# KhaoulaAguech/pl-fem-vectoriel

Measured on AMD Instinct MI355X. Metric: eigenmodes/sec (assembly+solve), 7-core P2 mesh, 10 modes; |Δn_eff| vs ref, higher is better.
Workload: dtype f64

## Files before the change

### pl_fem_vectoriel_amd/csrc/kernels_lanczos.hip

```cpp
#include <algorithm>
#include <cmath>
#include <functional>

#include "device.h"
#include "p2_element.h"

namespace plfem {
namespace {

typedef double v4d __attribute__((ext_vector_type(4)));
constexpr int CHUNK = PANEL_CHUNK;

__global__ __launch_bounds__(256) void k_scale_store(int64_t n, const double* __restrict__ w,
                                                     const double* __restrict__ bw, const double* __restrict__ beta2,
                                                     double* __restrict__ v, double* __restrict__ bv,
                                                     double* __restrict__ beta_out) {
  const double b2 = *beta2;
  const double beta = sqrt(fmax(b2, 0.0));
  const double inv = beta > 0.0 ? 1.0 / beta : 0.0;
  const int64_t i = (int64_t)blockIdx.x * 256 + threadIdx.x;
  if (i == 0 && beta_out) *beta_out = beta;
  if (i >= n) return;
  v[i] = w[i] * inv;
  bv[i] = bw[i] * inv;
}

__global__ __launch_bounds__(256) void k_axpby(int64_t n, double a, const double* __restrict__ x, double b,
                                               const double* __restrict__ y, double* __restrict__ z) {
  const int64_t i = (int64_t)blockIdx.x * 256 + threadIdx.x;
  if (i < n) z[i] = a * x[i] + b * y[i];
}

template <int P, int CW>
__global__ __launch_bounds__(256) void k_panel_dot_p(int64_t n, int ncols, int nchunks, const double* __restrict__ Pm,
                                                     const double* __restrict__ W, int64_t ldw,
                                                     double* __restrict__ partial) {
  const int c0 = (blockIdx.y * 4 + (threadIdx.x >> 6)) * CW;
  if (c0 >= ncols) return;
  const int lane = threadIdx.x & 63;
  const int64_t i0 = (int64_t)blockIdx.x * CHUNK;
  const int64_t i1 = min(n, i0 + CHUNK);
  const double* col[CW];
#pragma unroll
  for (int t = 0; t < CW; ++t) col[t] = Pm + (int64_t)min(c0 + t, ncols - 1) * n;
  double acc[CW][P];
#pragma unroll
  for (int t = 0; t < CW; ++t)
#pragma unroll
    for (int q = 0; q < P; ++q) acc[t][q] = 0.0;
  int64_t i = i0 + lane;
  for (; i + 64 < i1; i += 128) {
    double a[2][CW], w[2][P];
#pragma unroll
    for (int h = 0; h < 2; ++h) {
#pragma unroll
      for (int t = 0; t < CW; ++t) a[h][t] = col[t][i + 64 * h];
#pragma unroll
      for (int q = 0; q < P; ++q) w[h][q] = W[(int64_t)q * ldw + i + 64 * h];
    }
#pragma unroll
    for (int h = 0; h < 2; ++h)
#pragma unroll
      for (int t = 0; t < CW; ++t)
#pragma unroll
        for (int q = 0; q < P; ++q) acc[t][q] += a[h][t] * w[h][q];
  }
  for (; i < i1; i += 64) {
    double w[P];
#pragma unroll
    for (int q = 0; q < P; ++q) w[q] = W[(int64_t)q * ldw + i];
#pragma unroll
    for (int t = 0; t < CW; ++t) {
      const double a = col[t][i];
#pragma unroll
      for (int q = 0; q < P; ++q) acc[t][q] += a * w[q];
    }
  }
#pragma unroll
  for (int t = 0; t < CW; ++t) {
#pragma unroll
    for (int q = 0; q < P; ++q) {
      double v = acc[t][q];
      for (int off = 32; off >= 1; off >>= 1) v += __shfl_xor(v, off);
      if (lane == 0 && c0 + t < ncols) partial[((int64_t)(c0 + t) * P + q) * nchunks + blockIdx.x] = v;
    }
  }
}

__global__ __launch_bounds__(64) void k_panel_dot_finish_p(int P, int nchunks, const double* __restrict__ partial,
                                                           double* __restrict__ h, int ldh, double* __restrict__ hacc,
                                                           int ldacc) {
  const int cq = blockIdx.x;
  const int c = cq / P, q = cq % P;
  double acc = 0.0;
  for (int t = threadIdx.x; t < nchunks; t += 64) acc += partial[(int64_t)cq * nchunks + t];
  for (int off = 32; off >= 1; off >>= 1) acc += __shfl_xor(acc, off);
  if (threadIdx.x == 0) {
    h[c + (int64_t)q * ldh] = acc;
    if (hacc) hacc[c + (int64_t)q * ldacc] += acc;
  }
}

template <int P>
__global__ __launch_bounds__(256) void k_panel_axpy_p(int64_t n, int ncols, const double* __restrict__ Pm,
                                                      const double* __restrict__ H, int ldh, double* __restrict__ W,
                                                      int64_t ldw, double* __restrict__ wil, int N, int dpn) {
  extern __shared__ double sh[];
  for (int k = threadIdx.x; k < ncols * P; k += 256) sh[k] = H[(k / P) + (int64_t)(k % P) * ldh];
  __syncthreads();
  const int64_t i = (int64_t)blockIdx.x * 256 + threadIdx.x;
  if (i >= n) return;
  double acc[P];
#pragma unroll
  for (int q = 0; q < P; ++q) acc[q] = 0.0;
  for (int c = 0; c < ncols; ++c) {
    const double a = Pm[(int64_t)c * n + i];
#pragma unroll
    for (int q = 0; q < P; ++q) acc[q] += a * sh[c * P + q];
  }
  double w[P];
#pragma unroll
  for (int q = 0; q < P; ++q) {
    w[q] = W[(int64_t)q * ldw + i] - acc[q];
    W[(int64_t)q * ldw + i] = w[q];
  }
  if (wil) {
    const int comp = (int)(i / N), node = (int)(i - (int64_t)comp * N);
    double* d = wil + ((int64_t)node * dpn + comp) * P;
#pragma unroll
    for (int q = 0; q < P; ++q) d[q] = w[q];
  }
}


template <int P>
__global__ __launch_bounds__(FIRST_THREADS) void k_permute_dot_first(int64_t n2, int N, int nseg, int ncols, const int32_t* __restrict__ npos,
                                                          const double* __restrict__ xl, double* __restrict__ W, int64_t ldw,
                                                          const double* __restrict__ Pm, double* __restrict__ partial) {
  constexpr int CW = FIRST_COLS, V = CW * P, NT = FIRST_THREADS, NW = NT / 64;
  static_assert(V <= 64 && (V & (V - 1)) == 0 && FIRST_ROWS % NT == 0 && NW == 4, "multi_reduce<V>; whole rows per thread; four waves meet");
  __shared__ double red[NW][V];
  const int seg = blockIdx.x, wave = threadIdx.x >> 6, lane = threadIdx.x & 63;
  double acc[V];
#pragma unroll
  for (int v = 0; v < V; ++v) acc[v] = 0.0;
  const double* col[CW];
#pragma unroll
  for (int t = 0; t < CW; ++t) col[t] = Pm + (int64_t)min(t, ncols - 1) * n2;
  constexpr int RPT = FIRST_ROWS / NT;
  int64_t g[RPT];
  int pos[RPT];
  double a[RPT][CW], w[RPT][P];
#pragma unroll
  for (int j = 0; j < RPT; ++j) {
    g[j] = (int64_t)seg * FIRST_ROWS + j * NT + threadIdx.x;
    const bool on = g[j] < n2;
    const int c = on && g[j] >= N;
    pos[j] = on ? npos[(int)(g[j] - (int64_t)c * N)] : -1;
#pragma unroll
    for (int t = 0; t < CW; ++t) a[j][t] = on ? col[t][g[j]] : 0.0;
  }
#pragma unroll
  for (int j = 0; j < RPT; ++j) {
    const int c = g[j] >= N;
#pragma unroll
    for (int q = 0; q < P; ++q) w[j][q] = pos[j] >= 0 ? xl[((int64_t)pos[j] + c) * P + q] : 0.0;
  }
#pragma unroll
  for (int j = 0; j < RPT; ++j) {
    if (g[j] < n2) {
#pragma unroll
      for (int q = 0; q < P; ++q) W[(int64_t)q * ldw + g[j]] = w[j][q];
    }
#pragma unroll
    for (int t = 0; t < CW; ++t)
#pragma unroll
      for (int q = 0; q < P; ++q) acc[t * P + q] = fma(a[j][t], w[j][q], acc[t * P + q]);
  }
  multi_reduce<V, true>(acc, lane);
  if ((lane & (64 / V - 1)) == 0) red[wave][multi_reduce_index<V, true>(lane)] = acc[0];
  __syncthreads();
  if ((int)threadIdx.x < V) {
    const int v = threadIdx.x, t = v / P;
    if (t < ncols) partial[(int64_t)v * nseg + seg] = (red[0][v] + red[1][v]) + (red[2][v] + red[3][v]);
  }
}

template <int P>
__global__ __launch_bounds__(256) void k_axpy_first(int64_t n, int ncols, int nseg, const double* __restrict__ Pm,
                                                    const double* __restrict__ partial, double* __restrict__ Hout, int ldh,
                                                    double* __restrict__ W, int64_t ldw) {
  constexpr int CW = 8;
  __shared__ double sh[CW * P];
  {
    const int v = threadIdx.x >> 3, part = threadIdx.x & 7;
    double x = 0.0;
    if (v / P < ncols) {
      const double* pp = partial + (int64_t)v * nseg;
      int k = part;
      for (; k + 7 * 8 < nseg; k += 8 * 8) {
        double t[8];
#pragma unroll
        for (int u = 0; u < 8; ++u) t[u] = pp[k + 8 * u];
#pragma unroll
        for (int u = 0; u < 8; ++u) x += t[u];
      }
      for (; k < nseg; k += 8) x += pp[k];
    }
    x += __shfl_xor(x, 1, 8);
    x += __shfl_xor(x, 2, 8);
    x += __shfl_xor(x, 4, 8);
    if (part == 0) {
      sh[v] = x;
      if (blockIdx.x == 0 && v / P < ncols) Hout[(v / P) + (int64_t)(v % P) * ldh] = x;
    }
  }
  __syncthreads();
  const int64_t i = (int64_t)blockIdx.x * 256 + threadIdx.x;
  if (i >= n) return;
  double a[CW];
#pragma unroll
  for (int t = 0; t < CW; ++t) a[t] = Pm[(int64_t)min(t, ncols - 1) * n + i];
  double acc[P];
#pragma unroll
  for (int q = 0; q < P; ++q) acc[q] = 0.0;
#pragma unroll
  for (int t = 0; t < CW; ++t)
    if (t < ncols) {
#pragma unroll
      for (int q = 0; q < P; ++q) acc[q] = fma(a[t], sh[t * P + q], acc[q]);
    }
#pragma unroll
  for (int q = 0; q < P; ++q) W[(int64_t)q * ldw + i] -= acc[q];
}

template <int P>
__global__ __launch_bounds__(64 * P * P > 1024 ? 1024 : 64 * P * P) void k_chol_small(const double* __restrict__ G, int ldg, const double* __restrict__ partial,
                                                           int nchunks, double* __restrict__ Tblk, int ldT,
                                                           double* __restrict__ Rinv, int32_t* __restrict__ counters) {
  __shared__ double sG[P * P];
  if (G) {
    if (threadIdx.x < P * P) sG[threadIdx.x] = G[(threadIdx.x % P) + (int64_t)(threadIdx.x / P) * ldg];
  } else {
    const int lane = threadIdx.x & 63;
    for (int cq = threadIdx.x >> 6; cq < P * P; cq += blockDim.x >> 6) {
      const double* pp = partial + (int64_t)cq * nchunks;
      double acc = 0.0;
      int t = lane;
      for (; t + 7 * 64 < nchunks; t += 8 * 64) {
        double v[8];
#pragma unroll
        for (int u = 0; u < 8; ++u) v[u] = pp[t + 64 * u];
#pragma unroll
        for (int u = 0; u < 8; ++u) acc += v[u];
      }
      for (; t < nchunks; t += 64) acc += pp[t];
      for (int off = 32; off >= 1; off >>= 1) acc += __shfl_xor(acc, off);
      if (lane == 0) sG[(cq / P) + (cq % P) * P] = acc;
    }
  }
  __syncthreads();
  if (threadIdx.x != 0) return;
  ldg = P;
  G = sG;
  double R[P][P], X[P][P];
  for (int i = 0; i < P; ++i)
    for (int j = 0; j < P; ++j) { R[i][j] = 0.0; X[i][j] = 0.0; }
  for (int j = 0; j < P; ++j) {
    for (int i = 0; i <= j; ++i) {
      double v = 0.5 * (G[i + (int64_t)j * ldg] + G[j + (int64_t)i * ldg]);
      for (int k = 0; k < i; ++k) v -= R[k][i] * R[k][j];
      if (i == j) {
        if (!(v > 0.0)) { atomicAdd(&counters[2], 1); v = 1.0; }
        R[j][j] = sqrt(v);
      } else {
        R[i][j] = v / R[i][i];
      }
    }
  }
  for (int j = 0; j < P; ++j) {
    X[j][j] = 1.0 / R[j][j];
    for (int i = j - 1; i >= 0; --i) {
      double v = 0.0;
      for (int k = i + 1; k <= j; ++k) v -= R[i][k] * X[k][j];
      X[i][j] = v / R[i][i];
    }
  }
  for (int i = 0; i < P; ++i)
    for (int j = 0; j < P; ++j) {
      Tblk[i + (int64_t)j * ldT] = R[i][j];
      Rinv[i + j * P] = X[i][j];
    }
}

template <int P>
__global__ __launch_bounds__(256) void k_block_scale(int64_t n, const double* __restrict__ W, const double* __restrict__ BW,
                                                     int64_t ldw, const double* __restrict__ Rinv,
                                                     double* __restrict__ Vn, double* __restrict__ BVn, int64_t ldv,
                                                     const double* __restrict__ exp_src, int exp_n, double* __restrict__ exp_dst,
                                                     const int32_t* __restrict__ cnt_src, int32_t* __restrict__ cnt_dst,
                                                     double* __restrict__ bv_front, const int32_t* __restrict__ npos, int N) {
  __shared__ double X[P * P];
  if (threadIdx.x < P * P) X[threadIdx.x] = Rinv[threadIdx.x];
  if (blockIdx.x == 0 && exp_dst) {
    for (int t = threadIdx.x; t < exp_n; t += 256) exp_dst[t] = exp_src[t];
    if (threadIdx.x < 4) cnt_dst[threadIdx.x] = cnt_src[threadIdx.x];
  }
  __syncthreads();
  const int64_t i = (int64_t)blockIdx.x * 256 + threadIdx.x;
  if (i >= n) return;
  double w[P], bw[P];
#pragma unroll
  for (int q = 0; q < P; ++q) { w[q] = W[(int64_t)q * ldw + i]; bw[q] = BW[(int64_t)q * ldw + i]; }
  int64_t fo = -1;
  if (bv_front) {
    const int c = i >= N;
    const int pos = npos[(int)(i - (int64_t)c * N)];
    if (pos >= 0) fo = ((int64_t)pos + c) * P;
  }
#pragma unroll
  for (int q = 0; q < P; ++q) {
    double a = 0.0, b = 0.0;
#pragma unroll
    for (int k = 0; k <= q; ++k) { a += w[k] * X[k + q * P]; b += bw[k] * X[k + q * P]; }
    Vn[(int64_t)q * ldv + i] = a;
    BVn[(int64_t)q * ldv + i] = b;
    if (fo >= 0) bv_front[fo + q] = b;
  }
}

__global__ __launch_bounds__(256) void k_rotate(int64_t n, int m, int p, const double* __restrict__ V,
                                                const double* __restrict__ Smat, int ldS, double* __restrict__ out) {
  extern __shared__ double sS[];
  const int mpad = (m + 3) & ~3, ppad = (p + 15) & ~15;
  for (int k = threadIdx.x; k < mpad * ppad; k += 256) {
    int r = k / ppad, c = k % ppad;
    sS[k] = (r < m && c < p) ? Smat[(int64_t)c * ldS + r] : 0.0;
  }
  __syncthreads();
  const int wave = threadIdx.x >> 6, lane = threadIdx.x & 63;
  const int64_t i0 = ((int64_t)blockIdx.x * 4 + wave) * 16;
  if (i0 >= n) return;
  const int lr = lane & 15, lk = lane >> 4;
  const int64_t row = i0 + lr;
  const bool rv = row < n;
  for (int c0 = 0; c0 < ppad; c0 += 16) {
    v4d acc = (v4d){0.0, 0.0, 0.0, 0.0};
    for (int kk = 0; kk < mpad; kk += 4) {
      int k = kk + lk;
      double a = sS[k * ppad + c0 + lr];
      double b = (rv && k < m) ? V[(int64_t)k * n + row] : 0.0;
      acc = __builtin_amdgcn_mfma_f64_16x16x4f64(a, b, acc, 0, 0, 0);
    }
#pragma unroll
    for (int r = 0; r < 4; ++r) {
      int oc = c0 + lk + 4 * r;
      if (rv && oc < p) out[(int64_t)oc * n + row] = acc[r];
    }
  }
}

__global__ __launch_bounds__(256) void k_core_mask(int N, const double* __restrict__ doflocs,
                                                   const double* __restrict__ cores, int ncore,
                                                   const uint8_t* __restrict__ bmask, uint8_t* __restrict__ mask,
                                                   int32_t* __restrict__ counters) {
  const int i = blockIdx.x * 256 + threadIdx.x;
  bool counted = false;
  if (i < N) {
    const bool in = in_any_core(doflocs[i], doflocs[N + i], cores, ncore);
    mask[i] = in ? 1 : 0;
    counted = in && !bmask[i];
  }
  unsigned long long b = __ballot(counted);
  if ((threadIdx.x & 63) == 0 && b) atomicAdd(&counters[1], (int)__popcll(b));
}

constexpr int POST_MB = 4;
template <int DPN>
__global__ __launch_bounds__(256) void k_post_sums(int N, int k, int nblocks, const int32_t* __restrict__ rowptr,
                                                   const int32_t* __restrict__ colind, const double* __restrict__ dxx,
                                                   const double* __restrict__ dxy, const double* __restrict__ dyy,
                                                   const uint8_t* __restrict__ mask, const double* __restrict__ evecs,
                                                   double* __restrict__ partial) {
  constexpr int MB = POST_MB;
  const int mode0 = blockIdx.y * MB;
  const int nm = min(MB, k - mode0);
  const double* vx[MB];
#pragma unroll
  for (int j = 0; j < MB; ++j) vx[j] = evecs + (int64_t)min(mode0 + j, k - 1) * DPN * N;
// ... 367 lines not shown
```

### pl_fem_vectoriel_amd/csrc/kernels_sweep.hip

```cpp
#include <algorithm>

#include "device.h"

namespace plfem {
namespace {

struct SweepArgs {
  int leaf_level;
  int ldv;
  int sh;
  const int32_t *cinv0, *cinv1, *prow;
  const double* front;
  const double2* dinv2;
  double *fr, *u0, *u1, *ys, *xl;
};

template <int P, bool SOA>
__device__ __forceinline__ int sidx(int i, int u, int ldv) { return SOA ? u * ldv + i : i * P + u; }

template <int P>
struct FwdStage {
  double a[P], b0[P], b1[P];
  int c0, c1;
  __device__ __forceinline__ void request(const SweepArgs& A, int64_t np, int i, bool on) {
    c0 = c1 = -1;
#pragma unroll
    for (int u = 0; u < P; ++u) { a[u] = 0.0; b0[u] = 0.0; b1[u] = 0.0; }
    if (!on) return;
    const int64_t e = (2 * np + i) * P;
#pragma unroll
    for (int u = 0; u < P; ++u) a[u] = A.fr[e + u];
    if (!A.leaf_level) {
      c0 = A.cinv0[np + (i >> A.sh)];
      c1 = A.cinv1[np + (i >> A.sh)];
#pragma unroll
      for (int u = 0; u < P; ++u) { b0[u] = A.u0[e + u]; b1[u] = A.u1[e + u]; }
    }
  }
  __device__ __forceinline__ double value(int u) const {
    return a[u] + (c0 >= 0 ? b0[u] : 0.0) + (c1 >= 0 ? b1[u] : 0.0);
  }
};

template <int P, bool SOA>
__device__ __forceinline__ void stage_fwd(const SweepArgs& A, double* sv, int64_t np, int need, int T, int tid,
                                          FwdStage<P>& first) {
  for (int i = tid + T; i < need; i += T) {
    FwdStage<P> s;
    s.request(A, np, i, true);
#pragma unroll
    for (int u = 0; u < P; ++u) sv[sidx<P, SOA>(i, u, A.ldv)] = s.value(u);
  }
  first.request(A, np, tid, tid < need);
}

template <int P>
struct FwdOut {
  double w0[P], w1[P];
  int c0, c1;
  int64_t dst;
  __device__ __forceinline__ void request(const SweepArgs& A, int64_t npp, int64_t np, int s2, int m, int r) {
    c0 = c1 = -1;
    dst = -1;
#pragma unroll
    for (int u = 0; u < P; ++u) { w0[u] = 0.0; w1[u] = 0.0; }
    if (r >= m || r < s2) return;
    const int pr = A.prow[np + (r >> A.sh)];
    if (!A.leaf_level) {
      c0 = A.cinv0[np + (r >> A.sh)];
      c1 = A.cinv1[np + (r >> A.sh)];
      const int64_t e = (2 * np + r) * P;
#pragma unroll
      for (int u = 0; u < P; ++u) { w0[u] = A.u0[e + u]; w1[u] = A.u1[e + u]; }
    }
    if (pr >= 0) dst = (2 * npp + (pr << A.sh) + (r & A.sh)) * P;
  }
  __device__ __forceinline__ double w(int u) const { return (c0 >= 0 ? w0[u] : 0.0) + (c1 >= 0 ? w1[u] : 0.0); }
};

template <int P, int NW, int TBF>
__device__ __forceinline__ void fwd_tile_body(const SweepArgs& A, const SweepJob& J, double* __restrict__ sv, double* __restrict__ red) {
  const int f = J.f, m = J.m, s2 = J.s2;
  const int r0 = (J.rb & ~SWEEP_ROW_JOB_FLAG) * 64;
  const int64_t np = J.np;
  const int tid = threadIdx.x, wave = tid >> 6, lane = tid & 63;
  const int need = (r0 + 64 <= s2) ? r0 + 64 : s2;
  const int r = r0 + lane;
  const bool valid = r < m;
  const int h = lane >> 5, ra = r0 + 2 * (lane & 31), rb = ra + 1;
  const bool pvalid = ra < m;
  const int cea = pvalid ? ((ra < s2) ? ra + 1 : s2) : 0;
  const int ceb = pvalid ? ((rb < s2) ? rb + 1 : s2) : 0;
  const double* p = A.front + J.foff + ra;
  FwdOut<P> out;
  if (wave == 0) out.request(A, J.npp, np, s2, m, r);
  FwdStage<P> st;
  stage_fwd<P, false>(A, sv, np, need, NW * 64, tid, st);
  double2 a0[TBF];
#pragma unroll
  for (int t = 0; t < TBF; ++t) {
    const int c = 2 * (wave + NW * t) + h;
    a0[t] = (c < ceb) ? *reinterpret_cast<const double2*>(p + (int64_t)c * m) : make_double2(0.0, 0.0);
  }
  if (tid < need) {
#pragma unroll
    for (int u = 0; u < P; ++u) sv[tid * P + u] = st.value(u);
  }
  __syncthreads();
  double acc[2][P];
#pragma unroll
  for (int u = 0; u < P; ++u) { acc[0][u] = 0.0; acc[1][u] = 0.0; }
#pragma unroll
  for (int t = 0; t < TBF; ++t) {
    const int c = 2 * (wave + NW * t) + h;
    if (c < ceb) {
      const double ax = (c < cea) ? a0[t].x : 0.0;
#pragma unroll
      for (int u = 0; u < P; ++u) {
        const double v = sv[c * P + u];
        acc[0][u] += ax * v;
        acc[1][u] += a0[t].y * v;
      }
    }
  }
  for (int c0 = 2 * NW * TBF; c0 < ceb; c0 += 2 * NW * TBF) {
    double2 a[TBF];
#pragma unroll
    for (int t = 0; t < TBF; ++t) {
      const int c = c0 + 2 * (wave + NW * t) + h;
      a[t] = (c < ceb) ? *reinterpret_cast<const double2*>(p + (int64_t)c * m) : make_double2(0.0, 0.0);
    }
#pragma unroll
    for (int t = 0; t < TBF; ++t) {
      const int c = c0 + 2 * (wave + NW * t) + h;
      if (c < ceb) {
        const double ax = (c < cea) ? a[t].x : 0.0;
#pragma unroll
        for (int u = 0; u < P; ++u) {
          const double v = sv[c * P + u];
          acc[0][u] += ax * v;
          acc[1][u] += a[t].y * v;
        }
      }
    }
  }
#pragma unroll
  for (int u = 0; u < P; ++u) {
    acc[0][u] += __shfl_xor(acc[0][u], 32);
    acc[1][u] += __shfl_xor(acc[1][u], 32);
  }
  if (h == 0) {
#pragma unroll
    for (int u = 0; u < P; ++u)
      *reinterpret_cast<double2*>(&red[(wave * P + u) * 64 + 2 * lane]) = make_double2(acc[0][u], acc[1][u]);
  }
  __syncthreads();
  if (wave == 0 && valid) {
    double tot[P];
#pragma unroll
    for (int u = 0; u < P; ++u) {
      double t = 0.0;
#pragma unroll
      for (int w = 0; w < NW; ++w) t += red[(w * P + u) * 64 + lane];
      tot[u] = t;
    }
    if (r < s2) {
#pragma unroll
      for (int u = 0; u < P; ++u) A.ys[(2 * np + r) * P + u] = tot[u];
    } else if (out.dst >= 0) {
      double* d = ((f & 1) ? A.u0 : A.u1) + out.dst;
#pragma unroll
      for (int u = 0; u < P; ++u) d[u] = out.w(u) - tot[u];
    }
  }
}

template <int P, int NW, int R, int LOADS>
__device__ __forceinline__ void fwd_rows_body(const SweepArgs& A, const SweepJob& J, double* __restrict__ sv) {
  constexpr int RB = NW * R, UNR = LOADS / R, V = R * P;
  const int f = J.f, m = J.m, s2 = J.s2;
  const int j0 = (J.rb & ~SWEEP_ROW_JOB_FLAG) * RB;
  const int64_t np = J.np;
  const int tid = threadIdx.x, wave = tid >> 6, lane = tid & 63;
  const int need = min(s2, j0 + RB);
  const double* F = A.front + J.foff;
  int ce[R], cmax = 0;
  const double* rowp[R];
#pragma unroll
  for (int q = 0; q < R; ++q) {
    const int r = j0 + wave + NW * q;
    ce[q] = r < m ? ((r < s2) ? r + 1 : s2) : 0;
    cmax = max(cmax, ce[q]);
    rowp[q] = r < s2 ? F + (int64_t)r * m : F + (int64_t)m * s2 + (int64_t)(r - s2) * s2;
  }
  const int oidx = multi_reduce_index<V>(lane & (V - 1));
  const int orow = j0 + wave + NW * (oidx / P);
  FwdOut<P> out;
  out.request(A, J.npp, np, s2, m, lane < V ? orow : m);
  FwdStage<P> st;
  stage_fwd<P, true>(A, sv, np, need, NW * 64, tid, st);
  double2 a0[UNR][R];
#pragma unroll
  for (int t = 0; t < UNR; ++t) {
    const int i = 128 * t + 2 * lane;
#pragma unroll
    for (int q = 0; q < R; ++q) a0[t][q] = (i < ce[q]) ? *reinterpret_cast<const double2*>(rowp[q] + i) : make_double2(0.0, 0.0);
  }
  if (tid < need) {
#pragma unroll
    for (int u = 0; u < P; ++u) sv[u * A.ldv + tid] = st.value(u);
  }
  __syncthreads();
  double acc[V];
#pragma unroll
  for (int v = 0; v < V; ++v) acc[v] = 0.0;
#define PLFEM_FWD_ROWS_CONSUME(a, c)                                                                   \
  _Pragma("unroll") for (int t = 0; t < UNR; ++t) {                                                    \
    const int i = (c) + 128 * t + 2 * lane;                                                            \
    if (i < cmax) {                                                                                    \
      _Pragma("unroll") for (int u = 0; u < P; ++u) {                                                  \
        const double2 vi = *reinterpret_cast<const double2*>(&sv[u * A.ldv + i]);                      \
        _Pragma("unroll") for (int q = 0; q < R; ++q) {                                                \
          const double ay = (i + 1 < ce[q]) ? a[t][q].y : 0.0;                                         \
          acc[q * P + u] = fma(ay, vi.y, fma(a[t][q].x, vi.x, acc[q * P + u]));                        \
        }                                                                                              \
      }                                                                                                \
    }                                                                                                  \
  }
  PLFEM_FWD_ROWS_CONSUME(a0, 0)
  for (int c = 128 * UNR; c < cmax; c += 128 * UNR) {
    double2 a[UNR][R];
#pragma unroll
    for (int t = 0; t < UNR; ++t) {
      const int i = c + 128 * t + 2 * lane;
#pragma unroll
      for (int q = 0; q < R; ++q) a[t][q] = (i < ce[q]) ? *reinterpret_cast<const double2*>(rowp[q] + i) : make_double2(0.0, 0.0);
    }
    PLFEM_FWD_ROWS_CONSUME(a, c)
  }
#undef PLFEM_FWD_ROWS_CONSUME
  multi_reduce<V>(acc, lane);
  if (lane < V && orow < m) {
    const int u = oidx % P;
    if (orow < s2) {
      A.ys[(2 * np + orow) * P + u] = acc[0];
    } else if (out.dst >= 0) {
      double wu = out.w(0);
#pragma unroll
      for (int q = 1; q < P; ++q) wu = (u == q) ? out.w(q) : wu;
      (((f & 1) ? A.u0 : A.u1) + out.dst)[u] = wu - acc[0];
    }
  }
}

template <int P>
struct BwdStage {
  double v[P];
  int pr, i;
  bool own, on;
  __device__ __forceinline__ void request_index(const SweepArgs& A, int64_t np, int s2, int i_, bool on_) {
    i = i_;
    on = on_;
    own = i < s2;
    pr = -1;
    if (on && !own) pr = A.prow[np + (i >> A.sh)];
    if (on && own) {
      const double2 d = A.dinv2[2 * np + i];
#pragma unroll
      for (int u = 0; u < P; ++u) v[u] = fma(d.x, A.ys[(2 * np + i) * P + u], d.y * A.ys[(2 * np + (i ^ 1)) * P + u]);
    }
  }
  __device__ __forceinline__ void request_value(const SweepArgs& A, int64_t npp) {
    if (on && !own) {
#pragma unroll
      for (int u = 0; u < P; ++u) v[u] = pr >= 0 ? -A.xl[(2 * npp + (pr << A.sh) + (i & A.sh)) * P + u] : 0.0;
    }
  }
  template <bool SOA>
  __device__ __forceinline__ void finish(const SweepArgs& A, double* sv, int64_t np, bool publish) const {
    if (!on) return;
#pragma unroll
    for (int u = 0; u < P; ++u) sv[sidx<P, SOA>(i, u, A.ldv)] = v[u];
    if (publish && !own) {
#pragma unroll
      for (int u = 0; u < P; ++u) A.xl[(2 * np + i) * P + u] = -v[u];
    }
  }
};

template <int P, bool SOA>
__device__ __forceinline__ void stage_bwd_rest(const SweepArgs& A, double* sv, int lo, int m, int s2, int64_t np,
                                               int64_t npp, int T, int tid, bool publish) {
  for (int i = lo + tid + T; i < m; i += T) {
    BwdStage<P> s;
    s.request_index(A, np, s2, i, true);
    s.request_value(A, npp);
    s.template finish<SOA>(A, sv, np, publish);
  }
}

template <int P, int NW, int TBB>
__device__ __forceinline__ void bwd_tile_body(const SweepArgs& A, const SweepJob& J, double* __restrict__ sv, double* __restrict__ red) {
  const int rb = J.rb, m = J.m, s2 = J.s2;
  const int r0 = rb * 64;
  const int64_t np = J.np;
  const int64_t npp = J.npp;
  const int tid = threadIdx.x, wave = tid >> 6, lane = tid & 63;
  const bool publish = rb == 0 && !A.leaf_level;
  BwdStage<P> st;
  st.request_index(A, np, s2, r0 + tid, r0 + tid < m);
  const int r = r0 + lane;
  const bool valid = r < s2;
  const int h = lane >> 5, ra = r0 + 2 * (lane & 31);
  const bool pvalid = ra < s2;
  const double* p = A.front + J.foff + ra;
  const double* pz = A.front + J.foff + (int64_t)m * s2 + ra - (int64_t)s2 * s2;
  auto entry = [&](int i) { return *reinterpret_cast<const double2*>(i < s2 ? p + (int64_t)i * m : pz + (int64_t)i * s2); };
  const int cb = pvalid ? ra : m, ce = m;
  const int slot = 2 * wave + h;
  const int cstart = cb + ((slot - cb) & (2 * NW - 1));
  double2 a0[TBB];
#pragma unroll
  for (int t = 0; t < TBB; ++t) a0[t] = (cstart + 2 * NW * t < ce) ? entry(cstart + 2 * NW * t) : make_double2(0.0, 0.0);
  st.request_value(A, npp);
  stage_bwd_rest<P, false>(A, sv, r0, m, s2, np, npp, NW * 64, tid, publish);
  st.template finish<false>(A, sv, np, publish);
  __syncthreads();
  double acc[2][P];
#pragma unroll
  for (int u = 0; u < P; ++u) { acc[0][u] = 0.0; acc[1][u] = 0.0; }
#pragma unroll
  for (int t = 0; t < TBB; ++t) {
    const int c = cstart + 2 * NW * t;
    if (c < ce) {
      const double ay = (c > ra) ? a0[t].y : 0.0;
#pragma unroll
      for (int u = 0; u < P; ++u) {
        const double v = sv[c * P + u];
        acc[0][u] += a0[t].x * v;
        acc[1][u] += ay * v;
      }
    }
  }
  for (int c0 = cstart + 2 * NW * TBB; c0 < ce; c0 += 2 * NW * TBB) {
    double2 a[TBB];
#pragma unroll
    for (int t = 0; t < TBB; ++t) a[t] = (c0 + 2 * NW * t < ce) ? entry(c0 + 2 * NW * t) : make_double2(0.0, 0.0);
#pragma unroll
    for (int t = 0; t < TBB; ++t) {
      const int c = c0 + 2 * NW * t;
      if (c < ce) {
#pragma unroll
        for (int u = 0; u < P; ++u) {
          const double v = sv[c * P + u];
          acc[0][u] += a[t].x * v;
          acc[1][u] += a[t].y * v;
        }
      }
    }
  }
#pragma unroll
  for (int u = 0; u < P; ++u) {
    acc[0][u] += __shfl_xor(acc[0][u], 32);
    acc[1][u] += __shfl_xor(acc[1][u], 32);
  }
  if (h == 0) {
#pragma unroll
    for (int u = 0; u < P; ++u)
      *reinterpret_cast<double2*>(&red[(wave * P + u) * 64 + 2 * lane]) = make_double2(acc[0][u], acc[1][u]);
  }
  __syncthreads();
  if (wave == 0 && valid) {
#pragma unroll
    for (int u = 0; u < P; ++u) {
      double t = 0.0;
#pragma unroll
      for (int w = 0; w < NW; ++w) t += red[(w * P + u) * 64 + lane];
      A.xl[(2 * np + r) * P + u] = t;
    }
  }
}

template <int P, int NW, int R, int LOADS>
__device__ __forceinline__ void bwd_rows_body(const SweepArgs& A, const SweepJob& J, double* __restrict__ sv) {
  constexpr int RB = NW * R, UNR = LOADS / R, V = R * P;
  const int rb = J.rb, m = J.m, s2 = J.s2;
  const int j0 = rb * RB;
  const int64_t np = J.np;
  const int64_t npp = J.npp;
  const int tid = threadIdx.x, wave = tid >> 6, lane = tid & 63;
  const bool publish = rb == 0 && !A.leaf_level;
  const int lo = j0 & ~63;
  BwdStage<P> st;
  st.request_index(A, np, s2, lo + tid, lo + tid < m);
  const double* F = A.front + J.foff;
  int jq[R];
#pragma unroll
  for (int q = 0; q < R; ++q) {
    const int j = j0 + wave + NW * q;
    jq[q] = j < s2 ? j : m;
  }
  const int c0 = (j0 + wave) & ~63;
  double2 a0[UNR][R];
#pragma unroll
  for (int t = 0; t < UNR; ++t) {
    const int i = c0 + 128 * t + 2 * lane;
#pragma unroll
    for (int q = 0; q < R; ++q) a0[t][q] = (i < m && i + 1 >= jq[q]) ? *reinterpret_cast<const double2*>(F + i + (int64_t)jq[q] * m) : make_double2(0.0, 0.0);
  }
  st.request_value(A, npp);
  stage_bwd_rest<P, true>(A, sv, lo, m, s2, np, npp, NW * 64, tid, publish);
  st.template finish<true>(A, sv, np, publish);
  __syncthreads();
  const int oidx = multi_reduce_index<V>(lane & (V - 1));
  const int oj = j0 + wave + NW * (oidx / P);
  double acc[V];
#pragma unroll
  for (int v = 0; v < V; ++v) acc[v] = 0.0;
#define PLFEM_BWD_ROWS_CONSUME(a, c)                                                                   \
  _Pragma("unroll") for (int t = 0; t < UNR; ++t) {                                                    \
    const int i = (c) + 128 * t + 2 * lane;                                                            \
    if (i < m) {                                                                                       \
      _Pragma("unroll") for (int u = 0; u < P; ++u) {                                                  \
        const double2 vi = *reinterpret_cast<const double2*>(&sv[u * A.ldv + i]);                      \
        _Pragma("unroll") for (int q = 0; q < R; ++q) {                                                \
          const double ax = (i >= jq[q]) ? a[t][q].x : 0.0;                                            \
          acc[q * P + u] = fma(a[t][q].y, vi.y, fma(ax, vi.x, acc[q * P + u]));                        \
        }                                                                                              \
      }                                                                                                \
    }                                                                                                  \
  }
  PLFEM_BWD_ROWS_CONSUME(a0, c0)
  for (int c = c0 + 128 * UNR; c < m; c += 128 * UNR) {
    double2 a[UNR][R];
#pragma unroll
    for (int t = 0; t < UNR; ++t) {
      const int i = c + 128 * t + 2 * lane;
#pragma unroll
      for (int q = 0; q < R; ++q) a[t][q] = (i < m && i + 1 >= jq[q]) ? *reinterpret_cast<const double2*>(F + i + (int64_t)jq[q] * m) : make_double2(0.0, 0.0);
    }
    PLFEM_BWD_ROWS_CONSUME(a, c)
  }
#undef PLFEM_BWD_ROWS_CONSUME
  multi_reduce<V>(acc, lane);
  if (lane < V && oj < s2) A.xl[(2 * np + oj) * P + oidx % P] = acc[0];
}

template <int P, int R, int LD>
__global__ __launch_bounds__(512) void k_fwd_rows(const SweepJob* __restrict__ blk, SweepArgs A) {
  extern __shared__ __attribute__((aligned(16))) double sv[];
  const SweepJob job = blk[blockIdx.x];
  fwd_rows_body<P, 8, R, LD>(A, job, sv);
}

template <int P, int R, int LD>
__global__ __launch_bounds__(512) void k_bwd_rows(const SweepJob* __restrict__ blk, SweepArgs A) {
  extern __shared__ __attribute__((aligned(16))) double sv[];
  const SweepJob job = blk[blockIdx.x];
  bwd_rows_body<P, 8, R, LD>(A, job, sv);
}

template <int P, int LD>
__global__ __launch_bounds__(256) void k_fwd(const SweepJob* __restrict__ blk, SweepArgs A) {
  extern __shared__ __attribute__((aligned(16))) double sv[];
  __shared__ __attribute__((aligned(16))) double red[4 * P * 64];
  const SweepJob job = blk[blockIdx.x];
  fwd_tile_body<P, 4, LD>(A, job, sv, red);
}

template <int P, int LD>
__global__ __launch_bounds__(256) void k_fwd_mix(const SweepJob* __restrict__ blk, SweepArgs A) {
  extern __shared__ __attribute__((aligned(16))) double sv[];
  __shared__ __attribute__((aligned(16))) double red[4 * P * 64];
  const SweepJob job = blk[blockIdx.x];
  if (job.rb & SWEEP_ROW_JOB_FLAG) fwd_rows_body<P, 4, 4, LD>(A, job, sv);
  else fwd_tile_body<P, 4, LD>(A, job, sv, red);
}

template <int P, int LD>
__global__ __launch_bounds__(512) void k_bwd(const SweepJob* __restrict__ blk, SweepArgs A) {
  extern __shared__ __attribute__((aligned(16))) double sv[];
  __shared__ __attribute__((aligned(16))) double red[8 * P * 64];
  const SweepJob job = blk[blockIdx.x];
  bwd_tile_body<P, 8, LD>(A, job, sv, red);
}

template <int P>
__global__ __launch_bounds__(256) void k_permute_in(int64_t n2, int N, const int32_t* __restrict__ npos,
                                                    const double* __restrict__ rhs, int64_t ldx, double* __restrict__ fr) {
  const int64_t g = (int64_t)blockIdx.x * 256 + threadIdx.x;
  if (g >= n2) return;
  const int c = g >= N, node = (int)(g - (int64_t)c * N);
  const int pos = npos[node];
  if (pos < 0) return;
#pragma unroll
  for (int u = 0; u < P; ++u) fr[((int64_t)pos + c) * P + u] = rhs[(int64_t)u * ldx + g];
}

template <int P>
__global__ __launch_bounds__(256) void k_permute_out(int64_t n2, int N, const int32_t* __restrict__ npos,
                                                     const double* __restrict__ xl, double* __restrict__ x, int64_t ldx) {
  const int64_t g = (int64_t)blockIdx.x * 256 + threadIdx.x;
  if (g >= n2) return;
  const int c = g >= N, node = (int)(g - (int64_t)c * N);
  const int pos = npos[node];
#pragma unroll
  for (int u = 0; u < P; ++u) x[(int64_t)u * ldx + g] = pos >= 0 ? xl[((int64_t)pos + c) * P + u] : 0.0;
}

template <int P>
void sweeps(plfem_ctx* c) {
  hipStream_t st = c->stream;
  SweepArgs A;
  A.sh = c->sh;
  A.cinv0 = c->d_cinv0; A.cinv1 = c->d_cinv1; A.prow = c->d_prow;
  A.front = c->d_front; A.dinv2 = reinterpret_cast<const double2*>(c->d_delta);
  A.fr = c->d_fvec; A.u0 = c->d_u0; A.u1 = c->d_u1; A.ys = c->d_fvec2; A.xl = c->d_xl;
  const std::vector<LevelInfo>& levels = c->plan->levels;
  double sweep_total = 0.0;
  for (const LevelInfo& li : levels) sweep_total += li.sweep_bytes + 8.0 * (P - 1) * li.sweep_vec_doubles;
  const bool time_launches = c->prof_on && (c->prof_toggle++ & 1);
  const int pid_fwd = time_launches ? -1 : prof_open(c, PLFEM_PROF_FWD_SWEEP, sweep_total);
  for (int lev = c->L; lev >= 0; --lev) {
    const LevelInfo& li = levels[lev];
    if (li.fwd_n == 0) continue;
    A.leaf_level = lev == c->L ? 1 : 0;
    const SweepJob* blk = c->d_blk + li.fwd_off;
    A.ldv = sweep_ldv(li.max_s2);
    const size_t lds = sweep_dynamic_lds(P, li.max_s2);
    if (li.fwd_rows == 8) {
      hipLaunchKernelGGL((k_fwd_rows<P, 1, 4>), dim3(li.fwd_n), dim3(512), lds, st, blk, A);
    } else if (li.fwd_rows == 16) {
      hipLaunchKernelGGL((k_fwd_rows<P, 2, 4>), dim3(li.fwd_n), dim3(512), lds, st, blk, A);
    } else {
      const int pid = time_launches ? prof_open(c, PLFEM_PROF_KFWD, li.sweep_bytes + 8.0 * (P - 1) * li.sweep_vec_doubles) : -1;
      if (li.fwd_mixed) hipLaunchKernelGGL((k_fwd_mix<P, 4>), dim3(li.fwd_n), dim3(256), lds, st, blk, A);
      else hipLaunchKernelGGL((k_fwd<P, 4>), dim3(li.fwd_n), dim3(256), lds, st, blk, A);
      prof_close(c, pid);
    }
  }
  prof_close(c, pid_fwd);
  const int pid_bwd = time_launches ? -1 : prof_open(c, PLFEM_PROF_BWD_SWEEP, sweep_total);
  for (int lev = 0; lev <= c->L; ++lev) {
    const LevelInfo& li = levels[lev];
    if (li.bwd_n == 0) continue;
    A.leaf_level = lev == c->L ? 1 : 0;
    const SweepJob* blk = c->d_blk + li.bwd_off;
    A.ldv = sweep_ldv(li.max_m);
    const size_t lds = sweep_dynamic_lds(P, li.max_m);
    if (li.bwd_rows == 8)
      hipLaunchKernelGGL((k_bwd_rows<P, 1, 4>), dim3(li.bwd_n), dim3(512), lds, st, blk, A);
    else if (li.bwd_rows == 16)
      hipLaunchKernelGGL((k_bwd_rows<P, 2, 4>), dim3(li.bwd_n), dim3(512), lds, st, blk, A);
    else
      hipLaunchKernelGGL((k_bwd<P, 4>), dim3(li.bwd_n), dim3(512), lds, st, blk, A);
  }
  prof_close(c, pid_bwd);
}

}

void launch_solve(plfem_ctx* c, int P, const double* rhs, double* x, int64_t ldx, bool rhs_in_front_order) {
  const unsigned grid = (unsigned)((c->n2 + 255) / 256);
  with_constant<1, BLOCK_P>(P, [&](auto p) {
    constexpr int PT = decltype(p)::value;
    if (!rhs_in_front_order)
      hipLaunchKernelGGL(k_permute_in<PT>, dim3(grid), dim3(256), 0, c->stream, c->n2, c->N, c->d_npos, rhs, ldx, c->d_fvec);
    sweeps<PT>(c);
    if (x) hipLaunchKernelGGL(k_permute_out<PT>, dim3(grid), dim3(256), 0, c->stream, c->n2, c->N, c->d_npos, c->d_xl, x, ldx);
  });
}

void solve_refined(plfem_ctx* c, int P, const double* b, double* y, int64_t ld, bool b_in_front_order, int steps, double* ta,
                   double* tb, double* dy) {
  launch_solve(c, P, b, y, ld, b_in_front_order);
  const bool contiguous = ld == c->n2;
  const int nrun = contiguous ? 1 : P;
  const int64_t len = contiguous ? c->n2 * P : c->n2;
  auto axpby = [&](double a, const double* x, double bb, const double* yy, double* z) {
    for (int u = 0; u < nrun; ++u) launch_axpby(c, len, a, x + u * ld, bb, yy + u * ld, z + u * ld);
  };
  for (int it = 0; it < steps; ++it) {
    launch_spmv(c, 0, P, y, ta, ld);
    launch_spmv(c, 1, P, y, tb, ld);
    axpby(-1.0, ta, c->sigma, tb, ta);
    axpby(1.0, b, 1.0, ta, ta);
    launch_solve(c, P, ta, dy, ld);
    axpby(1.0, y, 1.0, dy, y);
  }
}

}
```

Measured before the change: 533.6.

## Issue sweep loads unconditionally with dummy addresses and delay waits via asm barriers

Sweep kernels now issue all global loads without branches, pointing inactive lanes at a valid dummy address and masking the values afterwards. Empty asm constraints mark where each value is first needed, so load waits happen late and the loads overlap with staging. Job descriptors are read with vector int4 loads pinned to scalar registers, and the backward staging is reordered. The panel-dot reduction now uses a shared multi-value shuffle reduction instead of one full butterfly per value. The cost is extra memory traffic for the dummy loads, more live registers, and reliance on how the compiler schedules waits.

Measured after the change: 546.3 (median of 6 runs). No clear change (+2.4%).

```diff
diff --git a/pl_fem_vectoriel_amd/csrc/kernels_lanczos.hip b/pl_fem_vectoriel_amd/csrc/kernels_lanczos.hip
--- a/pl_fem_vectoriel_amd/csrc/kernels_lanczos.hip
+++ b/pl_fem_vectoriel_amd/csrc/kernels_lanczos.hip
@@ -76,15 +76,15 @@
       for (int q = 0; q < P; ++q) acc[t][q] += a * w[q];
     }
   }
-#pragma unroll
-  for (int t = 0; t < CW; ++t) {
-#pragma unroll
-    for (int q = 0; q < P; ++q) {
-      double v = acc[t][q];
-      for (int off = 32; off >= 1; off >>= 1) v += __shfl_xor(v, off);
-      if (lane == 0 && c0 + t < ncols) partial[((int64_t)(c0 + t) * P + q) * nchunks + blockIdx.x] = v;
-    }
-  }
+  constexpr int V = CW * P;
+  double s[V];
+#pragma unroll
+  for (int t = 0; t < CW; ++t)
+#pragma unroll
+    for (int q = 0; q < P; ++q) s[t * P + q] = acc[t][q];
+  multi_reduce<V, true>(s, lane);
+  const int v = multi_reduce_index<V, true>(lane);
+  if ((lane & (64 / V - 1)) == 0 && c0 + v / P < ncols) partial[((int64_t)c0 * P + v) * nchunks + blockIdx.x] = s[0];
 }
 
 __global__ __launch_bounds__(64) void k_panel_dot_finish_p(int P, int nchunks, const double* __restrict__ partial,
diff --git a/pl_fem_vectoriel_amd/csrc/kernels_sweep.hip b/pl_fem_vectoriel_amd/csrc/kernels_sweep.hip
--- a/pl_fem_vectoriel_amd/csrc/kernels_sweep.hip
+++ b/pl_fem_vectoriel_amd/csrc/kernels_sweep.hip
@@ -18,25 +18,46 @@
 template <int P, bool SOA>
 __device__ __forceinline__ int sidx(int i, int u, int ldv) { return SOA ? u * ldv + i : i * P + u; }
 
+template <class T>
+__device__ __forceinline__ void landed(T& x) { asm volatile("" : "+v"(x)); }
+__device__ __forceinline__ void landed(double2& x) { asm volatile("" : "+v"(x.x), "+v"(x.y)); }
+template <int P>
+__device__ __forceinline__ void landed(double (&x)[P]) {
+#pragma unroll
+  for (int u = 0; u < P; ++u) landed(x[u]);
+}
+
+__device__ __forceinline__ SweepJob load_job(const SweepJob* __restrict__ blk) {
+  const int4* q = reinterpret_cast<const int4*>(blk + blockIdx.x);
+  int4 a = q[0], b = q[1], c = q[2];
+  asm volatile("" : "+s"(a.x), "+s"(a.y), "+s"(a.z), "+s"(a.w), "+s"(b.x), "+s"(b.y), "+s"(b.z), "+s"(b.w), "+s"(c.x), "+s"(c.y));
+  SweepJob J;
+  J.f = a.x; J.rb = a.y; J.m = a.z; J.s2 = a.w;
+  J.np = (int64_t)(((uint64_t)(uint32_t)b.y << 32) | (uint32_t)b.x);
+  J.npp = (int64_t)(((uint64_t)(uint32_t)b.w << 32) | (uint32_t)b.z);
+  J.foff = (int64_t)(((uint64_t)(uint32_t)c.y << 32) | (uint32_t)c.x);
+  J.reserved = 0;
+  return J;
+}
+
 template <int P>
 struct FwdStage {
   double a[P], b0[P], b1[P];
   int c0, c1;
   __device__ __forceinline__ void request(const SweepArgs& A, int64_t np, int i, bool on) {
+    const int ic = on ? i : 0;
+    const int64_t e = (2 * np + ic) * P;
     c0 = c1 = -1;
 #pragma unroll
-    for (int u = 0; u < P; ++u) { a[u] = 0.0; b0[u] = 0.0; b1[u] = 0.0; }
-    if (!on) return;
-    const int64_t e = (2 * np + i) * P;
-#pragma unroll
-    for (int u = 0; u < P; ++u) a[u] = A.fr[e + u];
+    for (int u = 0; u < P; ++u) { a[u] = A.fr[e + u]; b0[u] = 0.0; b1[u] = 0.0; }
     if (!A.leaf_level) {
-      c0 = A.cinv0[np + (i >> A.sh)];
-      c1 = A.cinv1[np + (i >> A.sh)];
+      c0 = A.cinv0[np + (ic >> A.sh)];
+      c1 = A.cinv1[np + (ic >> A.sh)];
 #pragma unroll
       for (int u = 0; u < P; ++u) { b0[u] = A.u0[e + u]; b1[u] = A.u1[e + u]; }
     }
   }
+  __device__ __forceinline__ void ready() { landed(c0); landed(c1); }
   __device__ __forceinline__ double value(int u) const {
     return a[u] + (c0 >= 0 ? b0[u] : 0.0) + (c1 >= 0 ? b1[u] : 0.0);
   }
@@ -48,6 +69,7 @@
   for (int i = tid + T; i < need; i += T) {
     FwdStage<P> s;
     s.request(A, np, i, true);
+    s.ready();
 #pragma unroll
     for (int u = 0; u < P; ++u) sv[sidx<P, SOA>(i, u, A.ldv)] = s.value(u);
   }
@@ -57,23 +79,27 @@
 template <int P>
 struct FwdOut {
   double w0[P], w1[P];
-  int c0, c1;
+  int c0, c1, pr;
+  bool on;
   int64_t dst;
-  __device__ __forceinline__ void request(const SweepArgs& A, int64_t npp, int64_t np, int s2, int m, int r) {
+  __device__ __forceinline__ void request(const SweepArgs& A, int64_t np, int r, bool on_) {
+    on = on_;
+    const int rc = on ? r : 0;
+    pr = A.prow[np + (rc >> A.sh)];
     c0 = c1 = -1;
-    dst = -1;
 #pragma unroll
     for (int u = 0; u < P; ++u) { w0[u] = 0.0; w1[u] = 0.0; }
-    if (r >= m || r < s2) return;
-    const int pr = A.prow[np + (r >> A.sh)];
     if (!A.leaf_level) {
-      c0 = A.cinv0[np + (r >> A.sh)];
-      c1 = A.cinv1[np + (r >> A.sh)];
-      const int64_t e = (2 * np + r) * P;
+      c0 = A.cinv0[np + (rc >> A.sh)];
+      c1 = A.cinv1[np + (rc >> A.sh)];
+      const int64_t e = (2 * np + rc) * P;
 #pragma unroll
       for (int u = 0; u < P; ++u) { w0[u] = A.u0[e + u]; w1[u] = A.u1[e + u]; }
     }
-    if (pr >= 0) dst = (2 * npp + (pr << A.sh) + (r & A.sh)) * P;
+  }
+  __device__ __forceinline__ void ready(const SweepArgs& A, int64_t npp, int r) {
+    landed(pr); landed(c0); landed(c1);
+    dst = (on && pr >= 0) ? (2 * npp + (pr << A.sh) + (r & A.sh)) * P : -1;
   }
   __device__ __forceinline__ double w(int u) const { return (c0 >= 0 ? w0[u] : 0.0) + (c1 >= 0 ? w1[u] : 0.0); }
 };
@@ -92,16 +118,20 @@
   const int cea = pvalid ? ((ra < s2) ? ra + 1 : s2) : 0;
   const int ceb = pvalid ? ((rb < s2) ? rb + 1 : s2) : 0;
   const double* p = A.front + J.foff + ra;
+  const double* ptile = A.front + J.foff + r0;
   FwdOut<P> out;
-  if (wave == 0) out.request(A, J.npp, np, s2, m, r);
+  const bool wave0 = __builtin_amdgcn_readfirstlane(wave) == 0;
+  if (wave0) out.request(A, np, r, r >= s2 && r < m);
   FwdStage<P> st;
   stage_fwd<P, false>(A, sv, np, need, NW * 64, tid, st);
   double2 a0[TBF];
 #pragma unroll
   for (int t = 0; t < TBF; ++t) {
     const int c = 2 * (wave + NW * t) + h;
-    a0[t] = (c < ceb) ? *reinterpret_cast<const double2*>(p + (int64_t)c * m) : make_double2(0.0, 0.0);
-  }
+    a0[t] = *reinterpret_cast<const double2*>((c < ceb) ? p + (int64_t)c * m : ptile);
+  }
+  if (wave0) out.ready(A, J.npp, r);
+  st.ready();
   if (tid < need) {
 #pragma unroll
     for (int u = 0; u < P; ++u) sv[tid * P + u] = st.value(u);
@@ -155,7 +185,7 @@
       *reinterpret_cast<double2*>(&red[(wave * P + u) * 64 + 2 * lane]) = make_double2(acc[0][u], acc[1][u]);
   }
   __syncthreads();
-  if (wave == 0 && valid) {
+  if (wave0 && valid) {
     double tot[P];
 #pragma unroll
     for (int u = 0; u < P; ++u) {
@@ -196,21 +226,30 @@
   const int oidx = multi_reduce_index<V>(lane & (V - 1));
   const int orow = j0 + wave + NW * (oidx / P);
   FwdOut<P> out;
-  out.request(A, J.npp, np, s2, m, lane < V ? orow : m);
+  out.request(A, np, orow, lane < V && orow >= s2 && orow < m);
   FwdStage<P> st;
   stage_fwd<P, true>(A, sv, np, need, NW * 64, tid, st);
+  const double* pblk = j0 < s2 ? F + (int64_t)j0 * m : F + (int64_t)m * s2 + (int64_t)(j0 - s2) * s2;
   double2 a0[UNR][R];
 #pragma unroll
   for (int t = 0; t < UNR; ++t) {
     const int i = 128 * t + 2 * lane;
 #pragma unroll
-    for (int q = 0; q < R; ++q) a0[t][q] = (i < ce[q]) ? *reinterpret_cast<const double2*>(rowp[q] + i) : make_double2(0.0, 0.0);
-  }
+    for (int q = 0; q < R; ++q) a0[t][q] = *reinterpret_cast<const double2*>((i < ce[q]) ? rowp[q] + i : pblk);
+  }
+  out.ready(A, J.npp, orow);
+  st.ready();
   if (tid < need) {
 #pragma unroll
     for (int u = 0; u < P; ++u) sv[u * A.ldv + tid] = st.value(u);
   }
   __syncthreads();
+#pragma unroll
+  for (int t = 0; t < UNR; ++t) {
+    const int i = 128 * t + 2 * lane;
+#pragma unroll
+    for (int q = 0; q < R; ++q) a0[t][q] = (i < ce[q]) ? a0[t][q] : make_double2(0.0, 0.0);
+  }
   double acc[V];
 #pragma unroll
   for (int v = 0; v < V; ++v) acc[v] = 0.0;
@@ -255,29 +294,36 @@
 
 template <int P>
 struct BwdStage {
-  double v[P];
+  double v[P], yp[P], x[P];
+  double2 d;
   int pr, i;
   bool own, on;
-  __device__ __forceinline__ void request_index(const SweepArgs& A, int64_t np, int s2, int i_, bool on_) {
+  __device__ __forceinline__ void request_index(const SweepArgs& A, int64_t np, int s2, int lo, int i_, bool on_) {
     i = i_;
     on = on_;
     own = i < s2;
-    pr = -1;
-    if (on && !own) pr = A.prow[np + (i >> A.sh)];
-    if (on && own) {
-      const double2 d = A.dinv2[2 * np + i];
-#pragma unroll
-      for (int u = 0; u < P; ++u) v[u] = fma(d.x, A.ys[(2 * np + i) * P + u], d.y * A.ys[(2 * np + (i ^ 1)) * P + u]);
-    }
-  }
-  __device__ __forceinline__ void request_value(const SweepArgs& A, int64_t npp) {
-    if (on && !own) {
-#pragma unroll
-      for (int u = 0; u < P; ++u) v[u] = pr >= 0 ? -A.xl[(2 * npp + (pr << A.sh) + (i & A.sh)) * P + u] : 0.0;
-    }
+    pr = A.prow[np + ((on ? i : lo) >> A.sh)];
+    const int io = (on && own) ? i : lo;
+    d = A.dinv2[2 * np + io];
+#pragma unroll
+    for (int u = 0; u < P; ++u) { v[u] = A.ys[(2 * np + io) * P + u]; yp[u] = A.ys[(2 * np + (io ^ 1)) * P + u]; }
+  }
+  __device__ __forceinline__ void request_value(const SweepArgs& A, int64_t npp, const double* xdummy) {
+    landed(pr);
+    const double* src = (on && !own && pr >= 0) ? A.xl + (2 * npp + (pr << A.sh) + (i & A.sh)) * P : xdummy;
+#pragma unroll
+    for (int u = 0; u < P; ++u) x[u] = src[u];
   }
   template <bool SOA>
-  __device__ __forceinline__ void finish(const SweepArgs& A, double* sv, int64_t np, bool publish) const {
+  __device__ __forceinline__ void finish(const SweepArgs& A, double* sv, int64_t np, bool publish) {
+    landed(d); landed(v); landed(yp);
+#pragma unroll
+    for (int u = 0; u < P; ++u) v[u] = fma(d.x, v[u], d.y * yp[u]);
+    landed(x);
+    if (!own) {
+#pragma unroll
+      for (int u = 0; u < P; ++u) v[u] = pr >= 0 ? -x[u] : 0.0;
+    }
     if (!on) return;
 #pragma unroll
     for (int u = 0; u < P; ++u) sv[sidx<P, SOA>(i, u, A.ldv)] = v[u];
@@ -288,13 +334,17 @@
   }
 };
 
+__device__ __forceinline__ const double* bwd_xdummy(const SweepArgs& A, const SweepJob& J, int P) {
+  return J.f ? A.xl + 2 * J.npp * P : A.ys + 2 * J.np * P;
+}
+
 template <int P, bool SOA>
 __device__ __forceinline__ void stage_bwd_rest(const SweepArgs& A, double* sv, int lo, int m, int s2, int64_t np,
-                                               int64_t npp, int T, int tid, bool publish) {
+                                               int64_t npp, const double* xdummy, int T, int tid, bool publish) {
   for (int i = lo + tid + T; i < m; i += T) {
     BwdStage<P> s;
-    s.request_index(A, np, s2, i, true);
-    s.request_value(A, npp);
+    s.request_index(A, np, s2, lo, i, true);
+    s.request_value(A, npp, xdummy);
     s.template finish<SOA>(A, sv, np, publish);
   }
 }
@@ -308,23 +358,27 @@
   const int tid = threadIdx.x, wave = tid >> 6, lane = tid & 63;
   const bool publish = rb == 0 && !A.leaf_level;
   BwdStage<P> st;
-  st.request_index(A, np, s2, r0 + tid, r0 + tid < m);
+  st.request_index(A, np, s2, r0, r0 + tid, r0 + tid < m);
+  const double* xdummy = bwd_xdummy(A, J, P);
   const int r = r0 + lane;
   const bool valid = r < s2;
   const int h = lane >> 5, ra = r0 + 2 * (lane & 31);
   const bool pvalid = ra < s2;
   const double* p = A.front + J.foff + ra;
   const double* pz = A.front + J.foff + (int64_t)m * s2 + ra - (int64_t)s2 * s2;
-  auto entry = [&](int i) { return *reinterpret_cast<const double2*>(i < s2 ? p + (int64_t)i * m : pz + (int64_t)i * s2); };
+  auto where = [&](int i) { return i < s2 ? p + (int64_t)i * m : pz + (int64_t)i * s2; };
+  auto entry = [&](int i) { return *reinterpret_cast<const double2*>(where(i)); };
+  const double* ptile = A.front + J.foff + r0 + (int64_t)r0 * m;
   const int cb = pvalid ? ra : m, ce = m;
   const int slot = 2 * wave + h;
   const int cstart = cb + ((slot - cb) & (2 * NW - 1));
   double2 a0[TBB];
 #pragma unroll
-  for (int t = 0; t < TBB; ++t) a0[t] = (cstart + 2 * NW * t < ce) ? entry(cstart + 2 * NW * t) : make_double2(0.0, 0.0);
-  st.request_value(A, npp);
-  stage_bwd_rest<P, false>(A, sv, r0, m, s2, np, npp, NW * 64, tid, publish);
+  for (int t = 0; t < TBB; ++t)
+    a0[t] = *reinterpret_cast<const double2*>((cstart + 2 * NW * t < ce) ? where(cstart + 2 * NW * t) : ptile);
+  st.request_value(A, npp, xdummy);
   st.template finish<false>(A, sv, np, publish);
+  stage_bwd_rest<P, false>(A, sv, r0, m, s2, np, npp, xdummy, NW * 64, tid, publish);
   __syncthreads();
   double acc[2][P];
 #pragma unroll
@@ -392,7 +446,8 @@
   const bool publish = rb == 0 && !A.leaf_level;
   const int lo = j0 & ~63;
   BwdStage<P> st;
-  st.request_index(A, np, s2, lo + tid, lo + tid < m);
+  st.request_index(A, np, s2, lo, lo + tid, lo + tid < m);
+  const double* xdummy = bwd_xdummy(A, J, P);
   const double* F = A.front + J.foff;
   int jq[R];
 #pragma unroll
@@ -401,17 +456,25 @@
     jq[q] = j < s2 ? j : m;
   }
   const int c0 = (j0 + wave) & ~63;
+  const double* pblk = F + (j0 & ~1) + (int64_t)j0 * m;
   double2 a0[UNR][R];
 #pragma unroll
   for (int t = 0; t < UNR; ++t) {
     const int i = c0 + 128 * t + 2 * lane;
 #pragma unroll
-    for (int q = 0; q < R; ++q) a0[t][q] = (i < m && i + 1 >= jq[q]) ? *reinterpret_cast<const double2*>(F + i + (int64_t)jq[q] * m) : make_double2(0.0, 0.0);
-  }
-  st.request_value(A, npp);
-  stage_bwd_rest<P, true>(A, sv, lo, m, s2, np, npp, NW * 64, tid, publish);
+    for (int q = 0; q < R; ++q)
+      a0[t][q] = *reinterpret_cast<const double2*>((i < m && i + 1 >= jq[q]) ? F + i + (int64_t)jq[q] * m : pblk);
+  }
+  st.request_value(A, npp, xdummy);
   st.template finish<true>(A, sv, np, publish);
+  stage_bwd_rest<P, true>(A, sv, lo, m, s2, np, npp, xdummy, NW * 64, tid, publish);
   __syncthreads();
+#pragma unroll
+  for (int t = 0; t < UNR; ++t) {
+    const int i = c0 + 128 * t + 2 * lane;
+#pragma unroll
+    for (int q = 0; q < R; ++q) a0[t][q] = (i < m && i + 1 >= jq[q]) ? a0[t][q] : make_double2(0.0, 0.0);
+  }
   const int oidx = multi_reduce_index<V>(lane & (V - 1));
   const int oj = j0 + wave + NW * (oidx / P);
   double acc[V];
@@ -449,14 +512,14 @@
 template <int P, int R, int LD>
 __global__ __launch_bounds__(512) void k_fwd_rows(const SweepJob* __restrict__ blk, SweepArgs A) {
   extern __shared__ __attribute__((aligned(16))) double sv[];
-  const SweepJob job = blk[blockIdx.x];
+  const SweepJob job = load_job(blk);
   fwd_rows_body<P, 8, R, LD>(A, job, sv);
 }
 
 template <int P, int R, int LD>
 __global__ __launch_bounds__(512) void k_bwd_rows(const SweepJob* __restrict__ blk, SweepArgs A) {
   extern __shared__ __attribute__((aligned(16))) double sv[];
-  const SweepJob job = blk[blockIdx.x];
+  const SweepJob job = load_job(blk);
   bwd_rows_body<P, 8, R, LD>(A, job, sv);
 }
 
@@ -464,7 +527,7 @@
 __global__ __launch_bounds__(256) void k_fwd(const SweepJob* __restrict__ blk, SweepArgs A) {
   extern __shared__ __attribute__((aligned(16))) double sv[];
   __shared__ __attribute__((aligned(16))) double red[4 * P * 64];
-  const SweepJob job = blk[blockIdx.x];
+  const SweepJob job = load_job(blk);
   fwd_tile_body<P, 4, LD>(A, job, sv, red);
 }
 
@@ -472,7 +535,7 @@
 __global__ __launch_bounds__(256) void k_fwd_mix(const SweepJob* __restrict__ blk, SweepArgs A) {
   extern __shared__ __attribute__((aligned(16))) double sv[];
   __shared__ __attribute__((aligned(16))) double red[4 * P * 64];
-  const SweepJob job = blk[blockIdx.x];
+  const SweepJob job = load_job(blk);
   if (job.rb & SWEEP_ROW_JOB_FLAG) fwd_rows_body<P, 4, 4, LD>(A, job, sv);
   else fwd_tile_body<P, 4, LD>(A, job, sv, red);
 }
@@ -481,7 +544,7 @@
 __global__ __launch_bounds__(512) void k_bwd(const SweepJob* __restrict__ blk, SweepArgs A) {
   extern __shared__ __attribute__((aligned(16))) double sv[];
   __shared__ __attribute__((aligned(16))) double red[8 * P * 64];
-  const SweepJob job = blk[blockIdx.x];
+  const SweepJob job = load_job(blk);
   bwd_tile_body<P, 8, LD>(A, job, sv, red);
 }
 
```
